# tsnorri/founder-sequences

Measured on AMD Instinct MI355X. Metric: alignment cells/s (m*n/T) through pBWT+DP, higher is better.
Workload: dtype u32

## Files before the change

### founder-sequences_amd/csrc/fseq_chainsort.hpp

```cpp
#pragma once

#include <type_traits>

#include "fseq_stream.hpp"
#include "fseq_types.hpp"

namespace fseq {

constexpr uint32_t CS_MAX_DIGIT_BITS = 9;
constexpr uint32_t CS_BINS = 1u << CS_MAX_DIGIT_BITS;
constexpr uint32_t CS_LEVELS = 16;

__host__ __device__ inline size_t chainsort_ws_words(uint32_t m)
{
	size_t const nblk = ((size_t) m + 63) / 64;
	return 8 * (size_t) m + CS_LEVELS * nblk + 64;
}

__device__ __forceinline__ uint64_t cs_match(uint32_t dg, bool in, uint32_t nbits)
{
	uint64_t mask = __ballot(in);
#pragma unroll
	for (uint32_t b = 0; b < CS_MAX_DIGIT_BITS; ++b)
		if (b < nbits)
		{
			uint64_t const bal = __ballot(in && ((dg >> b) & 1u));
			mask &= ((dg >> b) & 1u) ? bal : ~bal;
		}
	return mask;
}

__device__ __forceinline__ uint32_t cs_below(uint64_t mask)
{
	return (uint32_t) __builtin_amdgcn_mbcnt_hi((uint32_t) (mask >> 32), __builtin_amdgcn_mbcnt_lo((uint32_t) mask, 0u));
}

constexpr uint32_t P2_CLS_CAP = 11264;

constexpr uint32_t P2_RUN_CAP = 8832;
constexpr uint32_t P2_CLS_BITS = 14;
static_assert(P2_CLS_CAP <= (1u << P2_CLS_BITS), "a class of a reduced block fits a descriptor");

struct Pass2Lds {
	uint32_t scan[ST / WAVE + 1];
	uint32_t grp;
	union {
		struct {
			uint32_t hist[ST / WAVE][CS_BINS];
			uint32_t total[CS_BINS];
			uint16_t cls[P2_CLS_CAP];
		};
		struct {
			uint32_t off[P2_RUN_CAP + 1];
			uint32_t dsc[P2_RUN_CAP];
		};
	};
};

__host__ __device__ inline size_t pass2_lds_bytes() { return carve_bytes(1, sizeof(Pass2Lds)); }

__host__ __device__ inline size_t pass2_ws_r(uint32_t m) { return (((size_t) m + 1) / 2 + 3) & ~size_t(3); }
__host__ __device__ inline size_t pass2_ws_words(uint32_t m)
{
	size_t const nblk = ((size_t) m + 63) / 64;
	return pass2_ws_r(m) + 2 * (size_t) m + 2 * (size_t) m + 4 * (size_t) m + ((CS_LEVELS * nblk + 64 + 3) & ~size_t(3));
}
struct Pass2Ws {
	uint16_t *r;
	uint32_t *bufB, *bufA;
	uint4 *rec;
	uint32_t *tab;
};
__device__ __forceinline__ Pass2Ws pass2_ws(uint32_t *w, uint32_t m)
{
	Pass2Ws W;
	W.r = reinterpret_cast<uint16_t *>(w);
	W.bufB = w + pass2_ws_r(m);
	W.bufA = W.bufB + 2u * (size_t) m;
	W.rec = reinterpret_cast<uint4 *>(W.bufA + 2u * (size_t) m);
	W.tab = W.bufA + 6u * (size_t) m;
	return W;
}

__device__ __forceinline__ void pass2_digits(uint32_t D, uint32_t &npass, uint32_t &db)
{
	uint32_t bits = 1;
	while (bits < 32u && ((D - 1u) >> bits) != 0u) ++bits;
	npass = (bits + CS_MAX_DIGIT_BITS - 1u) / CS_MAX_DIGIT_BITS;
	db = (bits + npass - 1u) / npass;
}

template <typename PairT, uint32_t U = 4, typename Load0, typename KeyOf, typename Lds>
__device__ __forceinline__ void pass2_sort(uint32_t cnt, uint32_t npass, uint32_t db, Load0 load0, KeyOf key_of, PairT none, PairT *bufA, PairT *bufB, Lds &S)
{
	uint32_t const tid = threadIdx.x, lane = lane_id();
	uint32_t const wave = __builtin_amdgcn_readfirstlane(tid >> 6);
	constexpr uint32_t NW = ST / WAVE;
	uint32_t const nbins = 1u << db;
	uint32_t const per = ((cnt + NW - 1u) / NW + 63u) & ~63u;
	uint32_t const c_lo = min(cnt, wave * per), c_hi = min(cnt, c_lo + per);
	for (uint32_t p = 0; p < npass; ++p)
	{
		uint32_t const shift = p * db;
		bool const first = p == 0;
		PairT const *src = ((npass - p) & 1u) ? bufA : bufB;
		PairT *dst = ((npass - p) & 1u) ? bufB : bufA;
		auto load = [&](uint32_t i) -> PairT { return first ? load0(i) : src[i]; };
// ... 56 lines not shown
		}
#pragma unroll
		for (uint32_t u = 0; u < UB; ++u)
		{
			uint32_t const blk = b0 + u * NW, i = blk * 64u + lane;
			if (blk >= nblk) break;
			uint32_t const pre = wave_incl_max(v[u]);
			uint32_t const rev = (uint32_t) __builtin_amdgcn_ds_bpermute((int) ((63u - lane) << 2), (int) v[u]);
			uint32_t const sufr = wave_incl_max(rev);
			uint32_t const sufn = (uint32_t) __builtin_amdgcn_ds_bpermute((int) ((62u - min(lane, 62u)) << 2), (int) sufr);
			if (i < m) rec[i] = make_uint4(a[u], v[u], pre, lane == 63u ? 0u : sufn);
			if (lane == 63u) tab[blk] = pre;
		}
	}
	__syncthreads();
	for (uint32_t j = tid; j + 1u < nblk; j += ST) rec[j * 64u + 63u].w = tab[j + 1u];
	for (uint32_t k = 1; k < CS_LEVELS && (1u << k) <= nblk; ++k)
	{
		uint32_t const *lo = tab + (size_t) (k - 1u) * nblk;
		uint32_t *hi = tab + (size_t) k * nblk;
		for (uint32_t j = tid; j + (1u << k) <= nblk; j += ST) hi[j] = max(lo[j], lo[j + (1u << (k - 1u))]);
		__syncthreads();
	}
	__syncthreads();
}

__device__ __forceinline__ uint32_t pass2_range_max(uint32_t lo, uint32_t hi, uint4 const *rec, uint32_t const *tab, uint32_t nblk, uint32_t const *__restrict__ d0)
{
	uint32_t const bl = lo >> 6, bh = hi >> 6;
	uint4 const rc = rec[hi], q = rec[lo - 1u];
	uint32_t const pz = q.z, sv = q.w;
	uint32_t dv = max(sv, rc.z);
	if (bh > bl + 1u)
	{
		uint32_t const k = 31u - (uint32_t) __builtin_clz(bh - bl - 1u);
		uint32_t const *t = tab + (size_t) k * nblk;
		dv = max(dv, max(t[bl + 1u], t[bh - (1u << k)]));
	}
	if (bl == bh)
	{
		if ((lo & 63u) == 0u || rc.z > pz) dv = rc.z;
		else if ((hi & 63u) == 63u || sv > rc.w) dv = sv;
		else
		{
			dv = rc.y;
			for (uint32_t i = lo; i < hi; ++i) dv = max(dv, d0[i]);
		}
	}
	return dv;
}

__device__ __forceinline__ bool pass2_runs(
	uint32_t m, uint32_t const *__restrict__ kd, uint32_t D, Pass2Ws const &W, Pass2Lds &S, uint32_t run_cap, uint32_t *nrun,
	uint32_t const *__restrict__ a0, uint32_t const *__restrict__ d0, uint32_t *__restrict__ a1, uint32_t *__restrict__ d1)
{
	uint32_t const tid = threadIdx.x, lane = lane_id();
	uint32_t const wave = __builtin_amdgcn_readfirstlane(tid >> 6);
	constexpr uint32_t NW = ST / WAVE;
	uint16_t const *__restrict__ r = W.r;
	uint32_t pb = 1;
	while (pb < 32u && ((m - 1u) >> pb) != 0u) ++pb;
	uint32_t const pmask = (1u << pb) - 1u;
	uint32_t const nblk = (m + 63u) / 64u;
	uint32_t const per = ((m + NW - 1u) / NW + 63u) & ~63u;
	uint32_t const c_lo = min(m, wave * per), c_hi = min(m, c_lo + per);
	constexpr uint32_t U = 4;

	uint32_t npass, db;
	pass2_digits(D, npass, db);
	uint2 *const bufA = reinterpret_cast<uint2 *>(W.bufA), *const bufB = reinterpret_cast<uint2 *>(W.bufB);
	uint32_t *const pos_order = reinterpret_cast<uint32_t *>((npass & 1u) ? bufA : bufB);
	uint32_t R = 0, wbase = 0;
	for (uint32_t sweep = 0; sweep < 2u; ++sweep)
	{
		uint32_t prev = 0xFFFFFFFFu;
		if (c_lo > 0u && c_lo < c_hi) prev = (uint32_t) S.cls[r[c_lo - 1u]];
		uint32_t k0 = wbase;
		for (uint32_t i0 = c_lo; i0 < c_hi; i0 += 64u * U)
		{
			uint32_t rv[U];
#pragma unroll
			for (uint32_t u = 0; u < U; ++u) { uint32_t const i = i0 + u * 64u + lane; rv[u] = i < c_hi ? (uint32_t) r[i] : 0u; }
#pragma unroll
			for (uint32_t u = 0; u < U; ++u)
			{
				uint32_t const i = i0 + u * 64u + lane;
				if (i0 + u * 64u >= c_hi) break;
				bool const in = i < c_hi;
				uint32_t const cl = (uint32_t) S.cls[rv[u]];
				uint32_t const up = shfl_up_u32(cl, 1);
				bool const head = in && cl != (lane ? up : prev);
				uint64_t const heads = __ballot(head);
				if (sweep)
				{
					uint32_t const k = k0 + cs_below(heads);
					if (head)
					{
						pos_order[2u * k] = (cl << pb) | i;
						if (k) pos_order[2u * k - 1u] = i;
					}
				}
				k0 += (uint32_t) __popcll(heads);
				prev = readlane_u32(cl, 63);
			}
		}
		if (sweep) break;
		uint32_t const before = block_excl_add<ST>(lane == 0u ? k0 : 0u, S.scan, &R);
		wbase = __builtin_amdgcn_readfirstlane(before);
		*nrun = R;
		if (R > run_cap) return false;
	}
	if (tid == 0u) pos_order[2u * R - 1u] = m;
	__syncthreads();

	pass2_sort<uint2>(R, npass, db, [&](uint32_t i) -> uint2 { return reinterpret_cast<uint2 const *>(pos_order)[i]; },
	                  [&](uint2 x) -> uint32_t { return x.x >> pb; }, make_uint2(0u, 0u), bufA, bufB, S);
	{
		uint32_t const q = (R + ST - 1u) / ST, j0 = min(R, tid * q), j1 = min(R, j0 + q);
		uint32_t sum = 0;
		for (uint32_t j = j0; j < j1; ++j) { uint2 const x = bufB[j]; sum += x.y - (x.x & pmask); }
		uint32_t all;
		uint32_t at = block_excl_add<ST>(sum, S.scan, &all);
		for (uint32_t j = j0; j < j1; ++j) { uint2 const x = bufB[j]; S.off[j] = at; S.dsc[j] = x.x; at += x.y - (x.x & pmask); }
		if (tid == 0u) S.off[R] = m;
	}
	__syncthreads();

	uint32_t top = 1;
	while (top * 2u < R) top *= 2u;
	for (uint32_t p0 = tid; p0 < m; p0 += ST * U)
	{
		uint32_t jj[U], hh[U], av[U], dv[U];
#pragma unroll
		for (uint32_t u = 0; u < U; ++u)
		{
			uint32_t const p = min(p0 + u * ST, m - 1u);
			uint32_t j = 0;
			for (uint32_t step = top; step; step >>= 1) { uint32_t const t = j + step; if (t < R && S.off[t] <= p) j = t; }
			jj[u] = j;
			hh[u] = (S.dsc[j] & pmask) + (p - S.off[j]);
		}
#pragma unroll
		for (uint32_t u = 0; u < U; ++u) { av[u] = a0[hh[u]]; dv[u] = d0[hh[u]]; }
#pragma unroll
		for (uint32_t u = 0; u < U; ++u)
		{
			uint32_t const p = p0 + u * ST, j = jj[u];
			if (p >= m) break;
			if (S.off[j] == p)
			{
				uint32_t const me = S.dsc[j], pv = j ? S.dsc[j - 1u] : 0u;
				if (j == 0u || (pv >> pb) != (me >> pb)) dv[u] = kd[me >> pb];
				else dv[u] = pass2_range_max((pv & pmask) + (p - S.off[j - 1u]), hh[u], W.rec, W.tab, nblk, d0);
			}
			a1[p] = av[u];
			d1[p] = dv[u];
		}
	}
	__syncthreads();
	return true;
}

template <bool P4>
__device__ __forceinline__ void pass2_place(
	uint32_t m, uint32_t const *__restrict__ kd, std::conditional_t<P4, uint32_t, uint2> const *perm, uint4 const *rec, uint32_t const *tab,
	uint32_t const *__restrict__ d0, uint32_t *__restrict__ a1, uint32_t *__restrict__ d1)
{
	uint32_t const tid = threadIdx.x, lane = lane_id();
	using PairT = std::conditional_t<P4, uint32_t, uint2>;
	uint32_t pb = 1;
	while (pb < 32u && ((m - 1u) >> pb) != 0u) ++pb;
	uint32_t const pmask = pb < 32u ? (1u << pb) - 1u : 0xFFFFFFFFu;
	auto key_of = [&](PairT pr) -> uint32_t { if constexpr (P4) return pr >> pb; else return pr.x; };
	auto pos_of = [&](PairT pr) -> uint32_t { if constexpr (P4) return pr & pmask; else return pr.y; };
	uint32_t const nblk = (m + 63u) / 64u;
	{
		constexpr uint32_t U = 4;
		for (uint32_t p0 = tid; p0 < m; p0 += ST * U)
		{
			uint2 me[U], pv[U];
#pragma unroll
			for (uint32_t u = 0; u < U; ++u)
			{
				uint32_t const p = min(p0 + u * ST, m - 1u);
				PairT const pm_ = perm[p], pp_ = perm[p ? p - 1u : 0u];
				me[u] = make_uint2(key_of(pm_), pos_of(pm_));
				pv[u] = make_uint2(key_of(pp_), pos_of(pp_));
			}
			uint4 rc[U];
			uint32_t z0[U], w0[U], kdv[U], t0[U], t1[U];
#pragma unroll
			for (uint32_t u = 0; u < U; ++u)
			{
				uint32_t const p = p0 + u * ST;
				bool const first = p == 0u || pv[u].x != me[u].x;
				uint32_t const lo = pv[u].y + 1u, hi = me[u].y;
				uint32_t const bl = lo >> 6, bh = hi >> 6;
				rc[u] = rec[hi];
				z0[u] = 0u; w0[u] = 0u; kdv[u] = 0u; t0[u] = 0u; t1[u] = 0u;
				if (lane == 0u && !first) { uint4 const q = rec[pv[u].y]; z0[u] = q.z; w0[u] = q.w; }
				if (p < m && first) kdv[u] = kd[me[u].x];
				if (p < m && !first && bh > bl + 1u)
				{
					uint32_t const k = 31u - (uint32_t) __builtin_clz(bh - bl - 1u);
					uint32_t const *t = tab + (size_t) k * nblk;
					t0[u] = t[bl + 1u];
					t1[u] = t[bh - (1u << k)];
				}
			}
#pragma unroll
			for (uint32_t u = 0; u < U; ++u)
			{
// ... 14 lines not shown
						else if ((hi & 63u) == 63u || sv > rc[u].w) dv = sv;
						else
						{
							dv = rc[u].y;
							for (uint32_t i = lo; i < hi; i += 4u)
							{
								uint32_t const x0 = d0[i], x1 = i + 1u < hi ? d0[i + 1u] : 0u;
								uint32_t const x2 = i + 2u < hi ? d0[i + 2u] : 0u, x3 = i + 3u < hi ? d0[i + 3u] : 0u;
								dv = max(dv, max(max(x0, x1), max(x2, x3)));
							}
						}
					}
					a1[p] = rc[u].x;
					d1[p] = first ? kdv[u] : dv;
				}
			}
		}
	}
	__syncthreads();
}

template <bool P4>
__device__ __forceinline__ void pass2_step(
	uint32_t m, uint32_t const *__restrict__ kd, uint32_t D, Pass2Ws const &W, Pass2Lds &S,
	uint32_t const *__restrict__ d0, uint32_t *__restrict__ a1, uint32_t *__restrict__ d1)
{
	using PairT = std::conditional_t<P4, uint32_t, uint2>;
	uint32_t pb = 1;
	while (pb < 32u && ((m - 1u) >> pb) != 0u) ++pb;
	auto mk = [&](uint32_t key, uint32_t pos) -> PairT { if constexpr (P4) return (key << pb) | pos; else return make_uint2(key, pos); };
	auto key_of = [&](PairT pr) -> uint32_t { if constexpr (P4) return pr >> pb; else return pr.x; };
	uint16_t const *__restrict__ r = W.r;

	uint32_t npass, db;
	pass2_digits(D, npass, db);
	pass2_sort<PairT>(m, npass, db, [&](uint32_t i) -> PairT { return mk((uint32_t) S.cls[r[i]], i); }, key_of, mk(0u, 0u),
	                  reinterpret_cast<PairT *>(W.bufA), reinterpret_cast<PairT *>(W.bufB), S);
	pass2_place<P4>(m, kd, reinterpret_cast<PairT const *>(W.bufB), W.rec, W.tab, d0, a1, d1);
}

__global__ __launch_bounds__(ST) void k_chain_snap_grouped(
	uint32_t const *__restrict__ bstate_a, uint32_t const *__restrict__ bstate_d, uint32_t const *__restrict__ rank, uint32_t m,
	uint32_t const *__restrict__ task_blk, uint32_t const *__restrict__ cls, uint32_t const *__restrict__ headd, uint32_t const *__restrict__ ncls,
	uint32_t cap, uint2 const *__restrict__ grps, uint32_t ngrp, uint32_t *__restrict__ grp_next, uint32_t *__restrict__ snap_a,
	uint32_t *__restrict__ snap_d, uint32_t *ws, uint32_t run_cap, uint32_t *__restrict__ stats,
	uint16_t const *hand_keys, uint32_t const *hand_flag, uint32_t *hand_stats)
{
	extern __shared__ __attribute__((aligned(16))) char smem[];
	Pass2Lds &S = *reinterpret_cast<Pass2Lds *>(smem);
	uint32_t const tid = threadIdx.x;
	Pass2Ws const W0 = pass2_ws(ws + (size_t) blockIdx.x * pass2_ws_words(m), m);
	uint32_t pbits = 1;
	while (pbits < 32u && ((m - 1u) >> pbits) != 0u) ++pbits;
	for (;;)
	{
		if (tid == 0) S.grp = atomicAdd(grp_next, 1u);
		__syncthreads();
		uint32_t const g = S.grp;
		__syncthreads();
		if (g >= ngrp) break;
		uint2 const gr = grps[g];
		uint32_t const blk = task_blk[gr.x];
		size_t const sb = (size_t) blk * m;
		uint32_t const *a0 = bstate_a + sb, *d0 = bstate_d + sb;
		bool const handed = hand_keys != nullptr && hand_flag[blk] != 0u;
		Pass2Ws W = W0;
		if (handed) W.r = const_cast<uint16_t *>(hand_keys) + sb;
		if (hand_stats && tid == 0) atomicAdd(hand_stats + (handed ? 0 : 1), 1u);
		bool have_r = false;
		for (uint32_t task = gr.x; task < gr.x + gr.y; ++task)
		{
			uint32_t const D = ncls[task];
			if (D == 0xFFFFFFFFu) continue;
			size_t const ob = (size_t) task * m;
			if (D == 0u)
			{
				for (uint32_t i = tid; i < m; i += ST) { snap_a[ob + i] = a0[i]; snap_d[ob + i] = d0[i]; }
				if (tid == 0) atomicAdd(stats + 2, 1u);
				continue;
			}
			if (!have_r)
			{
				constexpr uint32_t U = 4;
				if (!handed)
					for (uint32_t i0 = tid; i0 < m; i0 += ST * U)
					{
						uint32_t rv[U];
#pragma unroll
						for (uint32_t u = 0; u < U; ++u) { uint32_t const i = i0 + u * ST; rv[u] = i < m ? rank[sb + a0[i]] : 0u; }
#pragma unroll
						for (uint32_t u = 0; u < U; ++u) { uint32_t const i = i0 + u * ST; if (i < m) W.r[i] = (uint16_t) rv[u]; }
					}
				pass2_records(m, a0, d0, W.rec, W.tab);
				have_r = true;
			}
			for (uint32_t j = tid; j < cap; j += ST) S.cls[j] = (uint16_t) cls[(size_t) task * cap + j];
			__syncthreads();
			uint32_t kb = 1;
			while (kb < 32u && ((D - 1u) >> kb) != 0u) ++kb;
			bool const p4 = kb + pbits <= 32u;
			uint32_t const *kd = headd + (size_t) task * cap;
			uint32_t nrun = 0;
			bool const by_runs = run_cap != 0u && P2_CLS_BITS + pbits <= 32u && pass2_runs(m, kd, D, W, S, run_cap, &nrun, a0, d0, snap_a + ob, snap_d + ob);
			if (!by_runs)
			{
				if (p4) pass2_step<true>(m, kd, D, W, S, d0, snap_a + ob, snap_d + ob);
				else pass2_step<false>(m, kd, D, W, S, d0, snap_a + ob, snap_d + ob);
			}
			if (tid == 0)
			{
				atomicAdd(stats + (by_runs ? 0 : 1), 1u);
				if (nrun)
				{
					atomicMax(stats + 3, nrun);
					atomicAdd(stats + 4 + min(P2_HIST - 1u, nrun > 1u ? 32u - (uint32_t) __builtin_clz(nrun - 1u) : 0u), 1u);
				}
			}
		}
	}
}

constexpr uint32_t CM_PART = 1024;
constexpr uint32_t CM_WG = 256;


struct CmWg { uint32_t x, chain; bool ok; };
__device__ __forceinline__ CmWg cm_wg(ChainMultiArgs const &A)
{
	CmWg w;
	uint32_t const nx = gridDim.x, L = blockIdx.y * nx + blockIdx.x;
	uint32_t const xcd = L & 7u, slot = L >> 3;
	w.chain = (slot / nx) * 8u + xcd;
	w.x = slot % nx;
	w.ok = w.chain < A.nchains;
	return w;
}

__host__ __device__ inline uint32_t chainmulti_parts(uint32_t m) { return (m + CM_PART - 1u) / CM_PART; }
__host__ __device__ inline uint32_t chainmulti_passes(uint32_t m)
{
	uint32_t bits = 1;
	while (bits < 32u && ((m - 1u) >> bits) != 0u) ++bits;
	return (bits + CS_MAX_DIGIT_BITS - 1u) / CS_MAX_DIGIT_BITS;
}

struct ChainMultiGeom {
	uint32_t b, npass, db, nbins;
	uint32_t pb;
	bool p4;
	bool active;
	uint32_t *w;
	uint32_t const *a0, *d0;
	uint32_t *a1, *d1;
	uint2 *pairA, *pairB;
	uint32_t *pm, *sm, *tab;
	uint32_t *hist;
};

__device__ __forceinline__ ChainMultiGeom chainmulti_geom(ChainMultiArgs const &A, uint32_t chain)
{
	ChainMultiGeom g;
	uint32_t const grp = chain + A.grp0;
	uint32_t const b0 = grp * A.G, b1 = min(A.nb_total, b0 + A.G);
	g.b = b0 + A.step;
	g.active = g.b < b1 && (A.out_rank != nullptr || g.b + 1u < b1 || g.b + 1u == A.nb_total);
	uint32_t const nk = g.active ? A.nkeys[g.b] : 1u;
	uint32_t bits = 1;
	while (bits < 32u && ((nk - 1u) >> bits) != 0u) ++bits;
	g.npass = (bits + CS_MAX_DIGIT_BITS - 1u) / CS_MAX_DIGIT_BITS;
	g.db = (bits + g.npass - 1u) / g.npass;
	g.nbins = 1u << g.db;
// ... 241 lines not shown
			dv = g.d0[hi];
			for (uint32_t i = lo; i < hi; ++i) dv = max(dv, g.d0[i]);
		}
		else
		{
			dv = max(g.sm[lo], g.pm[hi]);
			if (bh > bl + 1u)
			{
				uint32_t const k = 31u - (uint32_t) __builtin_clz(bh - bl - 1u);
				uint32_t const *t = g.tab + (size_t) k * nblk;
				dv = max(dv, max(t[bl + 1u], t[bh - (1u << k)]));
			}
		}
	}
	g.a1[p] = row; g.d1[p] = dv;
	uint32_t const grp = wg.chain + A.grp0;
	uint32_t const b1 = min(A.nb_total, grp * A.G + A.G);
	if (A.out_state_a && (g.b + 1u < b1 || g.b + 1u == A.nb_total))
	{
		A.out_state_a[(size_t) (g.b + 1u) * m + p] = row; A.out_state_d[(size_t) (g.b + 1u) * m + p] = dv;
	}
}

__global__ __launch_bounds__(ST) void k_cm_emit(ChainMultiArgs const A, uint32_t steps_done)
{
	extern __shared__ __attribute__((aligned(16))) char smem[];
	Carver cv{smem};
	StreamLds &L = *cv.take<StreamLds>(1);
	uint32_t const chain = blockIdx.x, grp = chain + A.grp0, m = A.m;
	uint32_t const b0 = grp * A.G;
	if (b0 >= A.nb_total) return;
	uint32_t const b1 = min(A.nb_total, b0 + A.G);
	uint32_t const cur = (b1 - b0) & 1u;
	(void) steps_done;
	uint32_t const *w = A.ws + (size_t) chain * chainsort_ws_words(m);
	uint32_t const *a = w + (size_t) cur * 2u * m, *d = a + m;
	uint32_t const kstart = (uint32_t) ((uint64_t) b0 * A.cols_per_block);
	stream_emit_ranks(m, a, d, kstart, A.out_rank + (size_t) grp * m, A.out_keyd + (size_t) grp * m, A.out_nkeys + grp, L.red);
}

constexpr uint32_t CW_RUN_CAP = 16384;
constexpr uint32_t CW_RBLK = CW_RUN_CAP / 64;
constexpr uint32_t CW_RLEVELS = 9;
static_assert(CW_RUN_CAP % 64u == 0u && CW_RBLK <= (1u << (CW_RLEVELS - 1u)), "the table over the blocks of runs");

struct ChainWgLds {
	uint32_t scan[ST / WAVE + 1];
	union {
		struct {
			uint32_t hist[ST / WAVE][CS_BINS];
			uint32_t total[CS_BINS];
		};
		struct {
			uint32_t off[CW_RUN_CAP + 1];
			uint32_t dlt[CW_RUN_CAP];
		};
	};
};
static_assert(sizeof(ChainWgLds) + 16u <= 160u * 1024u, "a workgroup a CU");

__host__ __device__ inline size_t chainwg_lds_bytes() { return carve_bytes(1, sizeof(ChainWgLds)); }

__host__ __device__ inline size_t chainwg_ws_rows(uint32_t m) { return ((size_t) m + 3) & ~size_t(3); }
__host__ __device__ inline size_t chainwg_ws_tab(uint32_t m) { return (CS_LEVELS * (((size_t) m + 63) / 64) + 64 + 3) & ~size_t(3); }
__host__ __device__ inline size_t chainwg_ws_words(uint32_t m)
{
	return 13 * chainwg_ws_rows(m) + chainwg_ws_tab(m) + 5 * (size_t) (CW_RUN_CAP + 64) + (size_t) CW_RLEVELS * CW_RBLK;
}
struct ChainWgWs {
	uint4 *rec;
	uint32_t *bufB, *bufA, *state, *keys, *tab;
	uint32_t *rstart, *rmax, *rpre, *rsuf, *rhead, *rtab;
};
__device__ __forceinline__ ChainWgWs chainwg_ws(uint32_t *w, uint32_t m)
{
	size_t const M = chainwg_ws_rows(m);
	ChainWgWs W;
	W.rec = reinterpret_cast<uint4 *>(w);
	W.bufB = w + 4 * M; W.bufA = w + 6 * M;
	W.state = w + 8 * M;
	W.keys = w + 12 * M;
	W.tab = w + 13 * M;
	W.rstart = W.tab + chainwg_ws_tab(m);
	W.rmax = W.rstart + (CW_RUN_CAP + 64); W.rpre = W.rmax + (CW_RUN_CAP + 64); W.rsuf = W.rpre + (CW_RUN_CAP + 64);
	W.rhead = W.rsuf + (CW_RUN_CAP + 64);
	W.rtab = W.rhead + (CW_RUN_CAP + 64);
	return W;
}

__device__ __forceinline__ uint32_t chainwg_rmax(uint32_t const *rmax, uint32_t k)
{
	return __hip_atomic_load(rmax + k, __ATOMIC_RELAXED, __HIP_MEMORY_SCOPE_AGENT);
}

__device__ __forceinline__ uint32_t chainwg_run_max(uint32_t lo, uint32_t hi, uint32_t R, ChainWgWs const &W)
{
	uint32_t const bl = lo >> 6, bh = hi >> 6;
	if (bl == bh)
	{
		if ((lo & 63u) == 0u) return W.rpre[hi];
		if ((hi & 63u) == 63u || hi + 1u == R) return W.rsuf[lo];
		uint32_t v = 0;
		for (uint32_t k = lo; k <= hi; ++k) v = max(v, chainwg_rmax(W.rmax, k));
		return v;
	}
	uint32_t v = max(W.rsuf[lo], W.rpre[hi]);
	if (bh > bl + 1u)
	{
		uint32_t const k = 31u - (uint32_t) __builtin_clz(bh - bl - 1u);
		uint32_t const *t = W.rtab + (size_t) k * CW_RBLK;
		v = max(v, max(t[bl + 1u], t[bh - (1u << k)]));
	}
	return v;
}


constexpr uint32_t CW_U = 8;

__device__ __forceinline__ uint32_t chainwg_keys(uint32_t m, uint32_t const *__restrict__ rk, uint32_t const *a0, ChainWgWs const &W, ChainWgLds &S, uint16_t *hk,
                                                 uint32_t *R)
{
	uint32_t const tid = threadIdx.x, lane = lane_id();
	uint32_t const wave = __builtin_amdgcn_readfirstlane(tid >> 6);
	constexpr uint32_t NW = ST / WAVE;
	uint32_t const per = ((m + NW - 1u) / NW + 63u) & ~63u;
	uint32_t const c_lo = min(m, wave * per), c_hi = min(m, c_lo + per);
	uint32_t prev = 0xFFFFFFFFu;
	if (c_lo > 0u && c_lo < c_hi) prev = rk[a0[c_lo - 1u]];
	uint32_t k0 = 0;
	for (uint32_t i0 = c_lo; i0 < c_hi; i0 += 64u * CW_U)
	{
		uint32_t av[CW_U], kv[CW_U];
#pragma unroll
		for (uint32_t u = 0; u < CW_U; ++u) { uint32_t const i = i0 + u * 64u + lane; av[u] = i < c_hi ? a0[i] : 0u; }
#pragma unroll
		for (uint32_t u = 0; u < CW_U; ++u) { uint32_t const i = i0 + u * 64u + lane; kv[u] = i < c_hi ? rk[av[u]] : 0u; }
#pragma unroll
		for (uint32_t u = 0; u < CW_U; ++u)
		{
			uint32_t const i = i0 + u * 64u + lane;
			if (i0 + u * 64u >= c_hi) break;
			bool const in = i < c_hi;
			if (in) W.keys[i] = kv[u];
			if (hk && in) hk[i] = (uint16_t) kv[u];
			uint32_t const up = shfl_up_u32(kv[u], 1);
			k0 += (uint32_t) __popcll(__ballot(in && kv[u] != (lane ? up : prev)));
			prev = readlane_u32(kv[u], 63);
		}
	}
	uint32_t const before = block_excl_add<ST>(lane == 0u ? k0 : 0u, S.scan, R);
	__syncthreads();
	return __builtin_amdgcn_readfirstlane(before);
}

__device__ __forceinline__ void chainwg_runs(
	uint32_t m, uint32_t const *__restrict__ kd, uint32_t nk, ChainWgWs const &W, ChainWgLds &S, uint32_t R, uint32_t wbase,
	uint32_t const *a0, uint32_t const *d0, uint32_t *a1, uint32_t *d1)
{
	uint32_t const tid = threadIdx.x, lane = lane_id();
	uint32_t const wave = __builtin_amdgcn_readfirstlane(tid >> 6);
	constexpr uint32_t NW = ST / WAVE;
	uint32_t const *keys = W.keys;
	uint32_t pb = 1;
	while (pb < 32u && ((m - 1u) >> pb) != 0u) ++pb;
	uint32_t const pmask = (1u << pb) - 1u;
	uint32_t const per = ((m + NW - 1u) / NW + 63u) & ~63u;
	uint32_t const c_lo = min(m, wave * per), c_hi = min(m, c_lo + per);
	uint32_t npass, db;
	pass2_digits(nk, npass, db);
	uint2 *const bufA = reinterpret_cast<uint2 *>(W.bufA), *const bufB = reinterpret_cast<uint2 *>(W.bufB);
	uint2 *const pos_order = (npass & 1u) ? bufA : bufB;

	for (uint32_t k = tid; k < R; k += ST) W.rmax[k] = 0u;
	__syncthreads();
	{
		uint32_t prev = 0xFFFFFFFFu;
		if (c_lo > 0u && c_lo < c_hi) prev = keys[c_lo - 1u];
		uint32_t k0 = wbase;
		for (uint32_t i0 = c_lo; i0 < c_hi; i0 += 64u * CW_U)
		{
			uint32_t kv[CW_U], dv[CW_U];
#pragma unroll
			for (uint32_t u = 0; u < CW_U; ++u)
			{
				uint32_t const i = i0 + u * 64u + lane;
				kv[u] = i < c_hi ? keys[i] : 0u;
				dv[u] = i < c_hi ? d0[i] : 0u;
			}
#pragma unroll
			for (uint32_t u = 0; u < CW_U; ++u)
			{
				uint32_t const i = i0 + u * 64u + lane;
				if (i0 + u * 64u >= c_hi) break;
				bool const in = i < c_hi;
				uint32_t const up = shfl_up_u32(kv[u], 1);
				bool const head = in && kv[u] != (lane ? up : prev);
				uint64_t const heads = __ballot(head);
				uint32_t const k = k0 + cs_below(heads) + (head ? 1u : 0u) - 1u;
				if (head) { pos_order[k] = make_uint2((kv[u] << pb) | i, k); W.rstart[k] = i; }
				uint64_t const upto = heads & (lane == 63u ? ~0ull : ((2ull << lane) - 1ull));
				uint32_t const s0 = upto ? 63u - (uint32_t) __builtin_clzll(upto) : 0u;
				uint32_t v = dv[u];
#pragma unroll
				for (uint32_t o = 1; o < 64u; o <<= 1)
				{
					uint32_t const t = shfl_up_u32(v, (int) o);
					if (lane >= s0 + o) v = max(v, t);
				}
				uint64_t const ins = __ballot(in);
				bool const last = in && (lane == 63u || !((ins >> (lane + 1u)) & 1ull) || ((heads >> (lane + 1u)) & 1ull));
				if (last) atomicMax(&W.rmax[k], v);
				k0 += (uint32_t) __popcll(heads);
				prev = readlane_u32(kv[u], 63);
			}
		}
	}
	if (tid == 0u) W.rstart[R] = m;
	__syncthreads();

	uint32_t const nrb = (R + 63u) / 64u;
	for (uint32_t blk = wave; blk < nrb; blk += NW)
	{
		uint32_t const k = blk * 64u + lane;
		uint32_t const v = k < R ? chainwg_rmax(W.rmax, k) : 0u;
		uint32_t const pre = wave_incl_max(v);
		uint32_t const rev = (uint32_t) __builtin_amdgcn_ds_bpermute((int) ((63u - lane) << 2), (int) v);
		uint32_t const sufr = wave_incl_max(rev);
		uint32_t const suf = (uint32_t) __builtin_amdgcn_ds_bpermute((int) ((63u - lane) << 2), (int) sufr);
		if (k < R) { W.rpre[k] = pre; W.rsuf[k] = suf; }
		if (lane == 63u) W.rtab[blk] = pre;
	}
	__syncthreads();
	for (uint32_t k = 1; k < CW_RLEVELS && (1u << k) <= nrb; ++k)
	{
		uint32_t const *lo = W.rtab + (size_t) (k - 1u) * CW_RBLK;
		uint32_t *hi = W.rtab + (size_t) k * CW_RBLK;
		for (uint32_t j = tid; j + (1u << k) <= nrb; j += ST) hi[j] = max(lo[j], lo[j + (1u << (k - 1u))]);
		__syncthreads();
	}

	pass2_sort<uint2>(R, npass, db, [&](uint32_t i) -> uint2 { return pos_order[i]; }, [&](uint2 x) -> uint32_t { return x.x >> pb; },
	                  make_uint2(0u, 0u), bufA, bufB, S);
	{
		constexpr uint32_t Q = CW_RUN_CAP / ST;
		static_assert(Q * ST == CW_RUN_CAP, "a thread's runs");
		uint32_t const q = (R + ST - 1u) / ST, j0 = min(R, tid * q), j1 = min(R, j0 + q);
		uint32_t st[Q], len[Q];
#pragma unroll
		for (uint32_t t = 0; t < Q; ++t)
		{
			uint2 const x = j0 + t < j1 ? bufB[j0 + t] : make_uint2(0u, 0u);
			st[t] = x.x & pmask; len[t] = x.y;
		}
#pragma unroll
		for (uint32_t t = 0; t < Q; ++t) len[t] = j0 + t < j1 ? W.rstart[len[t] + 1u] - st[t] : 0u;
		uint32_t sum = 0;
#pragma unroll
		for (uint32_t t = 0; t < Q; ++t) sum += len[t];
		uint32_t all;
		uint32_t at = block_excl_add<ST>(sum, S.scan, &all);
#pragma unroll
		for (uint32_t t = 0; t < Q; ++t)
			if (j0 + t < j1) { S.off[j0 + t] = at; S.dlt[j0 + t] = st[t] - at; at += len[t]; }
		if (tid == 0u) S.off[R] = m;
	}

	{
		constexpr uint32_t UH = 4;
		for (uint32_t j0 = tid; j0 < R; j0 += ST * UH)
		{
			uint2 me[UH], pv[UH];
			uint32_t hv[UH];
#pragma unroll
			for (uint32_t u = 0; u < UH; ++u)
			{
				uint32_t const j = min(j0 + u * ST, R - 1u);
				me[u] = bufB[j]; pv[u] = bufB[j ? j - 1u : 0u];
			}
#pragma unroll
			for (uint32_t u = 0; u < UH; ++u)
			{
				uint32_t const j = j0 + u * ST;
				hv[u] = 0u;
				if (j >= R) continue;
				if (j == 0u || (pv[u].x >> pb) != (me[u].x >> pb)) hv[u] = kd[me[u].x >> pb];
				else
				{
					hv[u] = d0[me[u].x & pmask];
					uint32_t const k_lo = pv[u].y + 1u, k_me = me[u].y;
					if (k_lo < k_me) hv[u] = max(hv[u], chainwg_run_max(k_lo, k_me - 1u, R, W));
				}
			}
#pragma unroll
			for (uint32_t u = 0; u < UH; ++u) { uint32_t const j = j0 + u * ST; if (j < R) W.rhead[j] = hv[u]; }
		}
	}
	__syncthreads();

	uint32_t top = 1;
	while (top * 2u < R) top *= 2u;
	for (uint32_t p0 = tid; p0 < m; p0 += ST * CW_U)
	{
		uint32_t jh[CW_U], hh[CW_U], av[CW_U], dv[CW_U];
#pragma unroll
		for (uint32_t u = 0; u < CW_U; ++u)
		{
			uint32_t const p = min(p0 + u * ST, m - 1u);
			uint32_t j = 0;
			for (uint32_t step = top; step; step >>= 1) { uint32_t const t = j + step; if (t < R && S.off[t] <= p) j = t; }
			hh[u] = p + S.dlt[j];
			jh[u] = S.off[j] == p ? j : 0xFFFFFFFFu;
		}
#pragma unroll
		for (uint32_t u = 0; u < CW_U; ++u) { av[u] = a0[hh[u]]; dv[u] = jh[u] != 0xFFFFFFFFu ? W.rhead[jh[u]] : d0[hh[u]]; }
#pragma unroll
		for (uint32_t u = 0; u < CW_U; ++u)
		{
			uint32_t const p = p0 + u * ST;
			if (p < m) { a1[p] = av[u]; d1[p] = dv[u]; }
		}
	}
	__syncthreads();
}

template <bool P4>
__device__ __forceinline__ void chainwg_sort(
	uint32_t m, uint32_t const *__restrict__ rk, uint32_t const *__restrict__ kd, uint32_t nk, ChainWgWs const &W, ChainWgLds &S, bool ident, uint32_t kstart,
	uint32_t const *a0, uint32_t const *d0, uint32_t *a1, uint32_t *d1)
{
	using PairT = std::conditional_t<P4, uint32_t, uint2>;
	uint32_t pb = 1;
	while (pb < 32u && ((m - 1u) >> pb) != 0u) ++pb;
	uint32_t const pmask = pb < 32u ? (1u << pb) - 1u : 0xFFFFFFFFu;
	auto mk = [&](uint32_t key, uint32_t pos) -> PairT { if constexpr (P4) return (key << pb) | pos; else return make_uint2(key, pos); };
	auto key_of = [&](PairT pr) -> uint32_t { if constexpr (P4) return pr >> pb; else return pr.x; };
	auto pos_of = [&](PairT pr) -> uint32_t { if constexpr (P4) return pr & pmask; else return pr.y; };
	uint32_t npass, db;
	pass2_digits(nk, npass, db);
	PairT *const bufA = reinterpret_cast<PairT *>(W.bufA), *const bufB = reinterpret_cast<PairT *>(W.bufB);
	if (ident)
	{
		pass2_sort<PairT, CW_U>(m, npass, db, [&](uint32_t i) -> PairT { return mk(rk[i], i); }, key_of, mk(0u, 0u), bufA, bufB, S);
		for (uint32_t p0 = threadIdx.x; p0 < m; p0 += ST * CW_U)
		{
			PairT me[CW_U], pv[CW_U];
			uint32_t dv[CW_U];
#pragma unroll
			for (uint32_t u = 0; u < CW_U; ++u) { uint32_t const p = min(p0 + u * ST, m - 1u); me[u] = bufB[p]; pv[u] = bufB[p ? p - 1u : 0u]; }
#pragma unroll
			for (uint32_t u = 0; u < CW_U; ++u)
			{
				uint32_t const p = p0 + u * ST;
				dv[u] = (p < m && (p == 0u || key_of(pv[u]) != key_of(me[u]))) ? kd[key_of(me[u])] : kstart;
			}
#pragma unroll
			for (uint32_t u = 0; u < CW_U; ++u) { uint32_t const p = p0 + u * ST; if (p < m) { a1[p] = pos_of(me[u]); d1[p] = dv[u]; } }
		}
		__syncthreads();
		return;
	}
	uint32_t const *keys = W.keys;
	pass2_records(m, a0, d0, W.rec, W.tab);
	pass2_sort<PairT, CW_U>(m, npass, db, [&](uint32_t i) -> PairT { return mk(keys[i], i); }, key_of, mk(0u, 0u), bufA, bufB, S);
	pass2_place<P4>(m, kd, bufB, W.rec, W.tab, d0, a1, d1);
}

__global__ __launch_bounds__(ST) void k_chain_wg(ChainMultiArgs const A, uint32_t *ws, uint32_t run_cap, uint32_t *stats)
{
	extern __shared__ __attribute__((aligned(16))) char smem[];
	ChainWgLds &S = *reinterpret_cast<ChainWgLds *>(smem);
	uint32_t const tid = threadIdx.x, m = A.m;
	ChainWgWs const W = chainwg_ws(ws + (size_t) blockIdx.x * chainwg_ws_words(m), m);
	uint32_t pbits = 1;
	while (pbits < 32u && ((m - 1u) >> pbits) != 0u) ++pbits;
	for (uint32_t chain = blockIdx.x; chain < A.nchains; chain += gridDim.x)
	{
		uint32_t const grp = chain + A.grp0;
		uint32_t const b0 = grp * A.G;
		if (b0 >= A.nb_total) continue;
		uint32_t const b1 = min(A.nb_total, b0 + A.G);
		uint32_t const kstart = (uint32_t) ((uint64_t) b0 * A.cols_per_block);
		bool ident = A.start_a == nullptr;
		uint32_t const *a0 = ident ? nullptr : A.start_a + (size_t) grp * m, *d0 = ident ? nullptr : A.start_d + (size_t) grp * m;
		if (A.out_state_a)
			for (uint32_t i = tid; i < m; i += ST)
			{
				A.out_state_a[(size_t) b0 * m + i] = ident ? i : a0[i];
				A.out_state_d[(size_t) b0 * m + i] = ident ? kstart : d0[i];
			}
		uint32_t pp = 0;
		for (uint32_t b = b0; b < b1; ++b)
		{
			bool const keep = b + 1u < b1 || b + 1u == A.nb_total;
			if (!A.out_rank && !keep) break;
			uint32_t *a1, *d1;
			if (A.out_state_a && keep) { a1 = A.out_state_a + (size_t) (b + 1u) * m; d1 = A.out_state_d + (size_t) (b + 1u) * m; }
			else { a1 = W.state + (size_t) pp * 2u * chainwg_ws_rows(m); d1 = a1 + chainwg_ws_rows(m); pp ^= 1u; }
			uint32_t const *rk = A.rank + (size_t) b * m, *kd = A.keyd + (size_t) b * m;
			uint32_t const nk = A.nkeys[b];
			uint32_t kb = 1;
			while (kb < 32u && ((nk - 1u) >> kb) != 0u) ++kb;
			bool const p4 = kb + pbits <= 32u;
			uint32_t nrun = 0;
			bool by_runs = false;
			uint16_t *const hk = A.hand_keys && A.out_state_a && !A.out_rank && !ident && nk <= 65536u ? A.hand_keys + (size_t) b * m : nullptr;
			if (!ident)
			{
				uint32_t R = 0;
				uint32_t const wbase = chainwg_keys(m, rk, a0, W, S, hk, &R);
				bool const may = run_cap != 0u && p4;
				nrun = may ? R : 0u;
				by_runs = may && R <= run_cap;
				if (by_runs) chainwg_runs(m, kd, nk, W, S, R, wbase, a0, d0, a1, d1);
			}
			if (!by_runs)
			{
				if (p4) chainwg_sort<true>(m, rk, kd, nk, W, S, ident, kstart, a0, d0, a1, d1);
				else chainwg_sort<false>(m, rk, kd, nk, W, S, ident, kstart, a0, d0, a1, d1);
			}
			if (hk && tid == 0u) A.hand_flag[b] = 1u;
			if (stats && tid == 0)
			{
				atomicAdd(stats + (ident ? 2 : by_runs ? 0 : 1), 1u);
				if (nrun)
				{
					atomicMax(stats + 3, nrun);
					atomicAdd(stats + 4 + min(P2_HIST - 1u, nrun > 1u ? 32u - (uint32_t) __builtin_clz(nrun - 1u) : 0u), 1u);
				}
			}
			ident = false;
			a0 = a1; d0 = d1;
		}
		if (A.out_rank)
		{
			stream_emit_ranks(m, a0, d0, kstart, A.out_rank + (size_t) grp * m, A.out_keyd + (size_t) grp * m, A.out_nkeys + grp, S.scan);
			__syncthreads();
		}
	}
}

}
```

Baseline: 2327 billion.

## Replace run binary search with LDS select bitmap and vectorize run-head sweep

Replaces the per-row binary search over run offsets with a bitmap of run starts plus per-64-row prefix counts in LDS, so each row finds its run with a popcount and mbcnt. In pass2_runs it also computes run-head d values once per run in a separate pass, and it reads the 16-bit class keys eight at a time with uint4 loads when aligned. Optional timestamp instrumentation is added behind a macro. The cost is extra LDS, an atomicOr per run and another barrier and sweep.

```diff
diff --git a/founder-sequences_amd/csrc/fseq_chainsort.hpp b/founder-sequences_amd/csrc/fseq_chainsort.hpp
--- a/founder-sequences_amd/csrc/fseq_chainsort.hpp
+++ b/founder-sequences_amd/csrc/fseq_chainsort.hpp
@@ -35,11 +35,69 @@
 	return (uint32_t) __builtin_amdgcn_mbcnt_hi((uint32_t) (mask >> 32), __builtin_amdgcn_mbcnt_lo((uint32_t) mask, 0u));
 }
 
+#ifdef FSEQ_RUN_STAMPS
+struct RunStamps {
+	unsigned long long last, acc[8];
+	uint32_t steps;
+	__device__ __forceinline__ void clear() { for (int i = 0; i < 8; ++i) acc[i] = 0; steps = 0; }
+	__device__ __forceinline__ void start() { last = __builtin_amdgcn_s_memrealtime(); }
+	__device__ __forceinline__ void mark(int part) { unsigned long long const t = __builtin_amdgcn_s_memrealtime(); acc[part] += t - last; last = t; }
+};
+#define FSEQ_RS_PARAM , RunStamps &rs
+#define FSEQ_RS_ARG , rs
+#define FSEQ_RS_MARK(part) rs.mark(part)
+#else
+#define FSEQ_RS_PARAM
+#define FSEQ_RS_ARG
+#define FSEQ_RS_MARK(part)
+#endif
+
 constexpr uint32_t P2_CLS_CAP = 11264;
 
 constexpr uint32_t P2_RUN_CAP = 8832;
 constexpr uint32_t P2_CLS_BITS = 14;
 static_assert(P2_CLS_CAP <= (1u << P2_CLS_BITS), "a class of a reduced block fits a descriptor");
+
+constexpr uint32_t CW_U = 8;
+
+constexpr uint32_t SEL_ROWS = 1u << 18;
+struct RunSelect {
+	uint32_t bits[SEL_ROWS / 32];
+	uint16_t pre[SEL_ROWS / 64];
+};
+
+__device__ __forceinline__ void sel_clear(RunSelect &B, uint32_t m)
+{
+	for (uint32_t w = threadIdx.x; w < 2u * ((m + 63u) / 64u); w += ST) B.bits[w] = 0u;
+}
+__device__ __forceinline__ void sel_set(RunSelect &B, uint32_t p) { atomicOr(&B.bits[p >> 5], 1u << (p & 31u)); }
+__device__ __forceinline__ void sel_scan(RunSelect &B, uint32_t m, uint32_t *scan)
+{
+	__syncthreads();
+	constexpr uint32_t Q = SEL_ROWS / 64u / ST;
+	uint32_t const nw = (m + 63u) / 64u, w0 = threadIdx.x * Q;
+	uint32_t c[Q], sum = 0;
+#pragma unroll
+	for (uint32_t t = 0; t < Q; ++t)
+	{
+		c[t] = w0 + t < nw ? (uint32_t) __popc(B.bits[2u * (w0 + t)]) + (uint32_t) __popc(B.bits[2u * (w0 + t) + 1u]) : 0u;
+		sum += c[t];
+	}
+	uint32_t all;
+	uint32_t at = block_excl_add<ST>(sum, scan, &all);
+#pragma unroll
+	for (uint32_t t = 0; t < Q; ++t)
+		if (w0 + t < nw) { B.pre[w0 + t] = (uint16_t) at; at += c[t]; }
+}
+__device__ __forceinline__ uint32_t sel_run(RunSelect const &B, uint32_t p, uint32_t m, bool *head)
+{
+	uint32_t const w = __builtin_amdgcn_readfirstlane(min(p, m - 1u) >> 6);
+	uint32_t const lo = __builtin_amdgcn_readfirstlane(B.bits[2u * w]), hi = __builtin_amdgcn_readfirstlane(B.bits[2u * w + 1u]);
+	uint32_t const lane = lane_id();
+	bool const h = (((lane < 32u ? lo : hi) >> (lane & 31u)) & 1u) != 0u;
+	*head = h;
+	return (uint32_t) B.pre[w] + (uint32_t) __builtin_amdgcn_mbcnt_hi(hi, __builtin_amdgcn_mbcnt_lo(lo, 0u)) + (h ? 1u : 0u) - 1u;
+}
 
 struct Pass2Lds {
 	uint32_t scan[ST / WAVE + 1];
@@ -51,8 +109,8 @@
 			uint16_t cls[P2_CLS_CAP];
 		};
 		struct {
-			uint32_t off[P2_RUN_CAP + 1];
-			uint32_t dsc[P2_RUN_CAP];
+			uint32_t dlt[P2_RUN_CAP];
+			RunSelect sel;
 		};
 	};
 };
@@ -215,7 +273,7 @@
 
 __device__ __forceinline__ bool pass2_runs(
 	uint32_t m, uint32_t const *__restrict__ kd, uint32_t D, Pass2Ws const &W, Pass2Lds &S, uint32_t run_cap, uint32_t *nrun,
-	uint32_t const *__restrict__ a0, uint32_t const *__restrict__ d0, uint32_t *__restrict__ a1, uint32_t *__restrict__ d1)
+	uint32_t const *__restrict__ a0, uint32_t const *__restrict__ d0, uint32_t *__restrict__ a1, uint32_t *__restrict__ d1 FSEQ_RS_PARAM)
 {
 	uint32_t const tid = threadIdx.x, lane = lane_id();
 	uint32_t const wave = __builtin_amdgcn_readfirstlane(tid >> 6);
@@ -229,6 +287,8 @@
 	uint32_t const c_lo = min(m, wave * per), c_hi = min(m, c_lo + per);
 	constexpr uint32_t U = 4;
 
+	bool const vec = (reinterpret_cast<uintptr_t>(r) & 15u) == 0u;
+	constexpr uint32_t PC = 8, UV = 4;
 	uint32_t npass, db;
 	pass2_digits(D, npass, db);
 	uint2 *const bufA = reinterpret_cast<uint2 *>(W.bufA), *const bufB = reinterpret_cast<uint2 *>(W.bufB);
@@ -239,7 +299,59 @@
 		uint32_t prev = 0xFFFFFFFFu;
 		if (c_lo > 0u && c_lo < c_hi) prev = (uint32_t) S.cls[r[c_lo - 1u]];
 		uint32_t k0 = wbase;
-		for (uint32_t i0 = c_lo; i0 < c_hi; i0 += 64u * U)
+		for (uint32_t i0 = c_lo; vec && i0 < c_hi; i0 += 64u * PC * UV)
+		{
+			uint4 rv[UV];
+#pragma unroll
+			for (uint32_t u = 0; u < UV; ++u)
+			{
+				uint32_t const ib = i0 + (u * 64u + lane) * PC;
+				rv[u] = make_uint4(0u, 0u, 0u, 0u);
+				if (ib + PC <= c_hi) rv[u] = *reinterpret_cast<uint4 const *>(r + ib);
+				else if (ib < c_hi)
+				{
+					uint32_t x[PC / 2u] = {0u, 0u, 0u, 0u};
+#pragma unroll
+					for (uint32_t e = 0; e < PC; ++e)
+						if (ib + e < c_hi) x[e >> 1] |= (uint32_t) r[ib + e] << (16u * (e & 1u));
+					rv[u] = make_uint4(x[0], x[1], x[2], x[3]);
+				}
+			}
+#pragma unroll
+			for (uint32_t u = 0; u < UV; ++u)
+			{
+				if (i0 + u * 64u * PC >= c_hi) break;
+				uint32_t const ib = i0 + (u * 64u + lane) * PC;
+				uint32_t const x[PC / 2u] = {rv[u].x, rv[u].y, rv[u].z, rv[u].w};
+				uint32_t cl[PC];
+#pragma unroll
+				for (uint32_t e = 0; e < PC; ++e) cl[e] = (uint32_t) S.cls[(x[e >> 1] >> (16u * (e & 1u))) & 0xFFFFu];
+				uint32_t const up = shfl_up_u32(cl[PC - 1u], 1);
+				uint32_t front = lane ? up : prev, hm = 0;
+#pragma unroll
+				for (uint32_t e = 0; e < PC; ++e)
+				{
+					if (ib + e < c_hi && cl[e] != front) hm |= 1u << e;
+					front = cl[e];
+				}
+				uint32_t const cnt = (uint32_t) __popc(hm), inc = wave_incl_add(cnt);
+				if (sweep)
+				{
+					uint32_t k = k0 + inc - cnt;
+#pragma unroll
+					for (uint32_t e = 0; e < PC; ++e)
+						if ((hm >> e) & 1u)
+						{
+							pos_order[2u * k] = (cl[e] << pb) | (ib + e);
+							if (k) pos_order[2u * k - 1u] = ib + e;
+							++k;
+						}
+				}
+				k0 += readlane_u32(inc, 63);
+				prev = readlane_u32(cl[PC - 1u], 63);
+			}
+		}
+		for (uint32_t i0 = c_lo; !vec && i0 < c_hi; i0 += 64u * U)
 		{
 			uint32_t rv[U];
 #pragma unroll
@@ -272,55 +384,87 @@
 		wbase = __builtin_amdgcn_readfirstlane(before);
 		*nrun = R;
 		if (R > run_cap) return false;
+		FSEQ_RS_MARK(1);
 	}
 	if (tid == 0u) pos_order[2u * R - 1u] = m;
 	__syncthreads();
+	FSEQ_RS_MARK(2);
 
 	pass2_sort<uint2>(R, npass, db, [&](uint32_t i) -> uint2 { return reinterpret_cast<uint2 const *>(pos_order)[i]; },
 	                  [&](uint2 x) -> uint32_t { return x.x >> pb; }, make_uint2(0u, 0u), bufA, bufB, S);
+	FSEQ_RS_MARK(3);
 	{
 		uint32_t const q = (R + ST - 1u) / ST, j0 = min(R, tid * q), j1 = min(R, j0 + q);
 		uint32_t sum = 0;
 		for (uint32_t j = j0; j < j1; ++j) { uint2 const x = bufB[j]; sum += x.y - (x.x & pmask); }
+		sel_clear(S.sel, m);
 		uint32_t all;
 		uint32_t at = block_excl_add<ST>(sum, S.scan, &all);
-		for (uint32_t j = j0; j < j1; ++j) { uint2 const x = bufB[j]; S.off[j] = at; S.dsc[j] = x.x; at += x.y - (x.x & pmask); }
-		if (tid == 0u) S.off[R] = m;
-	}
+		for (uint32_t j = j0; j < j1; ++j)
+		{
+			uint2 const x = bufB[j];
+			S.dlt[j] = (x.x & pmask) - at; sel_set(S.sel, at);
+			at += x.y - (x.x & pmask);
+		}
+		sel_scan(S.sel, m, S.scan);
+	}
+#ifdef FSEQ_RUN_STAMPS
 	__syncthreads();
-
-	uint32_t top = 1;
-	while (top * 2u < R) top *= 2u;
-	for (uint32_t p0 = tid; p0 < m; p0 += ST * U)
-	{
-		uint32_t jj[U], hh[U], av[U], dv[U];
-#pragma unroll
-		for (uint32_t u = 0; u < U; ++u)
-		{
-			uint32_t const p = min(p0 + u * ST, m - 1u);
-			uint32_t j = 0;
-			for (uint32_t step = top; step; step >>= 1) { uint32_t const t = j + step; if (t < R && S.off[t] <= p) j = t; }
-			jj[u] = j;
-			hh[u] = (S.dsc[j] & pmask) + (p - S.off[j]);
-		}
-#pragma unroll
-		for (uint32_t u = 0; u < U; ++u) { av[u] = a0[hh[u]]; dv[u] = d0[hh[u]]; }
-#pragma unroll
-		for (uint32_t u = 0; u < U; ++u)
-		{
-			uint32_t const p = p0 + u * ST, j = jj[u];
-			if (p >= m) break;
-			if (S.off[j] == p)
-			{
-				uint32_t const me = S.dsc[j], pv = j ? S.dsc[j - 1u] : 0u;
-				if (j == 0u || (pv >> pb) != (me >> pb)) dv[u] = kd[me >> pb];
-				else dv[u] = pass2_range_max((pv & pmask) + (p - S.off[j - 1u]), hh[u], W.rec, W.tab, nblk, d0);
-			}
-			a1[p] = av[u];
-			d1[p] = dv[u];
+#endif
+	FSEQ_RS_MARK(4);
+
+	uint32_t *const rhead = reinterpret_cast<uint32_t *>(bufA);
+	{
+		constexpr uint32_t UH = 4;
+		for (uint32_t j0 = tid; j0 < R; j0 += ST * UH)
+		{
+			uint2 me[UH], pv[UH];
+			uint32_t hv[UH];
+#pragma unroll
+			for (uint32_t u = 0; u < UH; ++u)
+			{
+				uint32_t const j = min(j0 + u * ST, R - 1u);
+				me[u] = bufB[j]; pv[u] = bufB[j ? j - 1u : 0u];
+			}
+#pragma unroll
+			for (uint32_t u = 0; u < UH; ++u)
+			{
+				uint32_t const j = j0 + u * ST;
+				hv[u] = 0u;
+				if (j >= R) continue;
+				if (j == 0u || (pv[u].x >> pb) != (me[u].x >> pb)) hv[u] = kd[me[u].x >> pb];
+				else hv[u] = pass2_range_max(pv[u].y, me[u].x & pmask, W.rec, W.tab, nblk, d0);
+			}
+#pragma unroll
+			for (uint32_t u = 0; u < UH; ++u) { uint32_t const j = j0 + u * ST; if (j < R) rhead[j] = hv[u]; }
 		}
 	}
 	__syncthreads();
+	FSEQ_RS_MARK(7);
+
+	for (uint32_t p0 = tid; p0 < m; p0 += ST * CW_U)
+	{
+		uint32_t jh[CW_U], hh[CW_U], av[CW_U], dv[CW_U];
+#pragma unroll
+		for (uint32_t u = 0; u < CW_U; ++u)
+		{
+			uint32_t const p = p0 + u * ST;
+			bool head;
+			uint32_t const j = sel_run(S.sel, p, m, &head);
+			hh[u] = p < m ? p + S.dlt[j] : 0u;
+			jh[u] = head && p < m ? j : 0xFFFFFFFFu;
+		}
+#pragma unroll
+		for (uint32_t u = 0; u < CW_U; ++u) { av[u] = a0[hh[u]]; dv[u] = jh[u] != 0xFFFFFFFFu ? rhead[jh[u]] : d0[hh[u]]; }
+#pragma unroll
+		for (uint32_t u = 0; u < CW_U; ++u)
+		{
+			uint32_t const p = p0 + u * ST;
+			if (p < m) { a1[p] = av[u]; d1[p] = dv[u]; }
+		}
+	}
+	__syncthreads();
+	FSEQ_RS_MARK(5);
 	return true;
 }
 
@@ -441,6 +585,10 @@
 	Pass2Ws const W0 = pass2_ws(ws + (size_t) blockIdx.x * pass2_ws_words(m), m);
 	uint32_t pbits = 1;
 	while (pbits < 32u && ((m - 1u) >> pbits) != 0u) ++pbits;
+#ifdef FSEQ_RUN_STAMPS
+	RunStamps rs;
+	uint32_t rs_groups = 0;
+#endif
 	for (;;)
 	{
 		if (tid == 0) S.grp = atomicAdd(grp_next, 1u);
@@ -457,6 +605,11 @@
 		if (handed) W.r = const_cast<uint16_t *>(hand_keys) + sb;
 		if (hand_stats && tid == 0) atomicAdd(hand_stats + (handed ? 0 : 1), 1u);
 		bool have_r = false;
+#ifdef FSEQ_RUN_STAMPS
+		rs.clear();
+		uint32_t rs_sorted = 0;
+		unsigned long long rs_runs = 0;
+#endif
 		for (uint32_t task = gr.x; task < gr.x + gr.y; ++task)
 		{
 			uint32_t const D = ncls[task];
@@ -480,17 +633,31 @@
 #pragma unroll
 						for (uint32_t u = 0; u < U; ++u) { uint32_t const i = i0 + u * ST; if (i < m) W.r[i] = (uint16_t) rv[u]; }
 					}
+#ifdef FSEQ_RUN_STAMPS
+				__syncthreads();
+				rs.start();
+#endif
 				pass2_records(m, a0, d0, W.rec, W.tab);
+				FSEQ_RS_MARK(6);
 				have_r = true;
 			}
+#ifdef FSEQ_RUN_STAMPS
+			RunStamps const rs_before = rs;
+			rs.start();
+#endif
 			for (uint32_t j = tid; j < cap; j += ST) S.cls[j] = (uint16_t) cls[(size_t) task * cap + j];
 			__syncthreads();
+			FSEQ_RS_MARK(0);
 			uint32_t kb = 1;
 			while (kb < 32u && ((D - 1u) >> kb) != 0u) ++kb;
 			bool const p4 = kb + pbits <= 32u;
 			uint32_t const *kd = headd + (size_t) task * cap;
 			uint32_t nrun = 0;
-			bool const by_runs = run_cap != 0u && P2_CLS_BITS + pbits <= 32u && pass2_runs(m, kd, D, W, S, run_cap, &nrun, a0, d0, snap_a + ob, snap_d + ob);
+			bool const by_runs = run_cap != 0u && P2_CLS_BITS + pbits <= 32u && pass2_runs(m, kd, D, W, S, run_cap, &nrun, a0, d0, snap_a + ob, snap_d + ob FSEQ_RS_ARG);
+#ifdef FSEQ_RUN_STAMPS
+			if (by_runs) { ++rs.steps; rs_runs += nrun; }
+			else { rs = rs_before; ++rs_sorted; }
+#endif
 			if (!by_runs)
 			{
 				if (p4) pass2_step<true>(m, kd, D, W, S, d0, snap_a + ob, snap_d + ob);
@@ -506,6 +673,13 @@
 				}
 			}
 		}
+#ifdef FSEQ_RUN_STAMPS
+		if (tid == 0 && (blockIdx.x & 63u) == 0u && rs.steps != 0u && rs_groups++ < 3u)
+			printf("p2 run stamps workgroup %u block %u (%u rows, %s keys, %u tasks by runs of %llu runs on average, %u sorted): records %llu, per task by runs: class table %llu, "
+			       "sweep 0 %llu, sweep 1 %llu, descriptor sort %llu, prefix sums %llu, heads %llu, output sweep %llu (x 10 ns)\n",
+			       blockIdx.x, blk, m, handed ? "handed-over" : "gathered", rs.steps, rs_runs / rs.steps, rs_sorted, rs.acc[6], rs.acc[0] / rs.steps, rs.acc[1] / rs.steps,
+			       rs.acc[2] / rs.steps, rs.acc[3] / rs.steps, rs.acc[4] / rs.steps, rs.acc[7] / rs.steps, rs.acc[5] / rs.steps);
+#endif
 	}
 }
 
@@ -853,7 +1027,10 @@
 			uint32_t total[CS_BINS];
 		};
 		struct {
-			uint32_t off[CW_RUN_CAP + 1];
+			union {
+				RunSelect sel;
+				uint32_t off[CW_RUN_CAP + 1];
+			};
 			uint32_t dlt[CW_RUN_CAP];
 		};
 	};
@@ -916,7 +1093,6 @@
 }
 
 
-constexpr uint32_t CW_U = 8;
 
 __device__ __forceinline__ uint32_t chainwg_keys(uint32_t m, uint32_t const *__restrict__ rk, uint32_t const *a0, ChainWgWs const &W, ChainWgLds &S, uint16_t *hk,
                                                  uint32_t *R)
@@ -956,7 +1132,7 @@
 
 __device__ __forceinline__ void chainwg_runs(
 	uint32_t m, uint32_t const *__restrict__ kd, uint32_t nk, ChainWgWs const &W, ChainWgLds &S, uint32_t R, uint32_t wbase,
-	uint32_t const *a0, uint32_t const *d0, uint32_t *a1, uint32_t *d1)
+	uint32_t const *a0, uint32_t const *d0, uint32_t *a1, uint32_t *d1 FSEQ_RS_PARAM)
 {
 	uint32_t const tid = threadIdx.x, lane = lane_id();
 	uint32_t const wave = __builtin_amdgcn_readfirstlane(tid >> 6);
@@ -971,6 +1147,7 @@
 	pass2_digits(nk, npass, db);
 	uint2 *const bufA = reinterpret_cast<uint2 *>(W.bufA), *const bufB = reinterpret_cast<uint2 *>(W.bufB);
 	uint2 *const pos_order = (npass & 1u) ? bufA : bufB;
+	bool const by_select = m <= SEL_ROWS;
 
 	for (uint32_t k = tid; k < R; k += ST) W.rmax[k] = 0u;
 	__syncthreads();
@@ -1018,6 +1195,7 @@
 	}
 	if (tid == 0u) W.rstart[R] = m;
 	__syncthreads();
+	FSEQ_RS_MARK(1);
 
 	uint32_t const nrb = (R + 63u) / 64u;
 	for (uint32_t blk = wave; blk < nrb; blk += NW)
@@ -1039,9 +1217,11 @@
 		for (uint32_t j = tid; j + (1u << k) <= nrb; j += ST) hi[j] = max(lo[j], lo[j + (1u << (k - 1u))]);
 		__syncthreads();
 	}
+	FSEQ_RS_MARK(2);
 
 	pass2_sort<uint2>(R, npass, db, [&](uint32_t i) -> uint2 { return pos_order[i]; }, [&](uint2 x) -> uint32_t { return x.x >> pb; },
 	                  make_uint2(0u, 0u), bufA, bufB, S);
+	FSEQ_RS_MARK(3);
 	{
 		constexpr uint32_t Q = CW_RUN_CAP / ST;
 		static_assert(Q * ST == CW_RUN_CAP, "a thread's runs");
@@ -1058,13 +1238,23 @@
 		uint32_t sum = 0;
 #pragma unroll
 		for (uint32_t t = 0; t < Q; ++t) sum += len[t];
+		if (by_select) sel_clear(S.sel, m);
 		uint32_t all;
 		uint32_t at = block_excl_add<ST>(sum, S.scan, &all);
 #pragma unroll
 		for (uint32_t t = 0; t < Q; ++t)
-			if (j0 + t < j1) { S.off[j0 + t] = at; S.dlt[j0 + t] = st[t] - at; at += len[t]; }
-		if (tid == 0u) S.off[R] = m;
-	}
+			if (j0 + t < j1)
+			{
+				if (by_select) sel_set(S.sel, at); else S.off[j0 + t] = at;
+				S.dlt[j0 + t] = st[t] - at; at += len[t];
+			}
+		if (by_select) sel_scan(S.sel, m, S.scan);
+		else if (tid == 0u) S.off[R] = m;
+	}
+#ifdef FSEQ_RUN_STAMPS
+	__syncthreads();
+#endif
+	FSEQ_RS_MARK(4);
 
 	{
 		constexpr uint32_t UH = 4;
@@ -1097,20 +1287,36 @@
 		}
 	}
 	__syncthreads();
+	FSEQ_RS_MARK(5);
 
 	uint32_t top = 1;
 	while (top * 2u < R) top *= 2u;
 	for (uint32_t p0 = tid; p0 < m; p0 += ST * CW_U)
 	{
 		uint32_t jh[CW_U], hh[CW_U], av[CW_U], dv[CW_U];
-#pragma unroll
-		for (uint32_t u = 0; u < CW_U; ++u)
-		{
-			uint32_t const p = min(p0 + u * ST, m - 1u);
-			uint32_t j = 0;
-			for (uint32_t step = top; step; step >>= 1) { uint32_t const t = j + step; if (t < R && S.off[t] <= p) j = t; }
-			hh[u] = p + S.dlt[j];
-			jh[u] = S.off[j] == p ? j : 0xFFFFFFFFu;
+		if (by_select)
+		{
+#pragma unroll
+			for (uint32_t u = 0; u < CW_U; ++u)
+			{
+				uint32_t const p = p0 + u * ST;
+				bool head;
+				uint32_t const j = sel_run(S.sel, p, m, &head);
+				hh[u] = p < m ? p + S.dlt[j] : 0u;
+				jh[u] = head && p < m ? j : 0xFFFFFFFFu;
+			}
+		}
+		else
+		{
+#pragma unroll
+			for (uint32_t u = 0; u < CW_U; ++u)
+			{
+				uint32_t const p = min(p0 + u * ST, m - 1u);
+				uint32_t j = 0;
+				for (uint32_t step = top; step; step >>= 1) { uint32_t const t = j + step; if (t < R && S.off[t] <= p) j = t; }
+				hh[u] = p + S.dlt[j];
+				jh[u] = S.off[j] == p ? j : 0xFFFFFFFFu;
+			}
 		}
 #pragma unroll
 		for (uint32_t u = 0; u < CW_U; ++u) { av[u] = a0[hh[u]]; dv[u] = jh[u] != 0xFFFFFFFFu ? W.rhead[jh[u]] : d0[hh[u]]; }
@@ -1122,6 +1328,7 @@
 		}
 	}
 	__syncthreads();
+	FSEQ_RS_MARK(6);
 }
 
 template <bool P4>
@@ -1174,6 +1381,9 @@
 	ChainWgWs const W = chainwg_ws(ws + (size_t) blockIdx.x * chainwg_ws_words(m), m);
 	uint32_t pbits = 1;
 	while (pbits < 32u && ((m - 1u) >> pbits) != 0u) ++pbits;
+#ifdef FSEQ_RUN_STAMPS
+	RunStamps rs;
+#endif
 	for (uint32_t chain = blockIdx.x; chain < A.nchains; chain += gridDim.x)
 	{
 		uint32_t const grp = chain + A.grp0;
@@ -1181,6 +1391,10 @@
 		if (b0 >= A.nb_total) continue;
 		uint32_t const b1 = min(A.nb_total, b0 + A.G);
 		uint32_t const kstart = (uint32_t) ((uint64_t) b0 * A.cols_per_block);
+#ifdef FSEQ_RUN_STAMPS
+		rs.clear();
+		unsigned long long rs_runs = 0;
+#endif
 		bool ident = A.start_a == nullptr;
 		uint32_t const *a0 = ident ? nullptr : A.start_a + (size_t) grp * m, *d0 = ident ? nullptr : A.start_d + (size_t) grp * m;
 		if (A.out_state_a)
@@ -1208,11 +1422,20 @@
 			if (!ident)
 			{
 				uint32_t R = 0;
+#ifdef FSEQ_RUN_STAMPS
+				RunStamps const rs_before = rs;
+				rs.start();
+#endif
 				uint32_t const wbase = chainwg_keys(m, rk, a0, W, S, hk, &R);
+				FSEQ_RS_MARK(0);
 				bool const may = run_cap != 0u && p4;
 				nrun = may ? R : 0u;
 				by_runs = may && R <= run_cap;
-				if (by_runs) chainwg_runs(m, kd, nk, W, S, R, wbase, a0, d0, a1, d1);
+				if (by_runs) chainwg_runs(m, kd, nk, W, S, R, wbase, a0, d0, a1, d1 FSEQ_RS_ARG);
+#ifdef FSEQ_RUN_STAMPS
+				if (by_runs) { ++rs.steps; rs_runs += R; }
+				else rs = rs_before;
+#endif
 			}
 			if (!by_runs)
 			{
@@ -1232,6 +1455,13 @@
 			ident = false;
 			a0 = a1; d0 = d1;
 		}
+#ifdef FSEQ_RUN_STAMPS
+		if (tid == 0 && (blockIdx.x & 63u) == 0u && chain == blockIdx.x && rs.steps != 0u)
+			printf("cw run stamps workgroup %u chain %u (%u rows, %s, %u steps by runs of %llu runs on average), per step by runs: keys and run count %llu, "
+			       "a descriptors and maxima %llu, b table %llu, c descriptor sort %llu, prefix sums %llu, d heads %llu, e new order %llu (x 10 ns)\n",
+			       blockIdx.x, chain, m, A.out_rank ? "composition" : "expansion", rs.steps, rs_runs / rs.steps, rs.acc[0] / rs.steps, rs.acc[1] / rs.steps,
+			       rs.acc[2] / rs.steps, rs.acc[3] / rs.steps, rs.acc[4] / rs.steps, rs.acc[5] / rs.steps, rs.acc[6] / rs.steps);
+#endif
 		if (A.out_rank)
 		{
 			stream_emit_ranks(m, a0, d0, kstart, A.out_rank + (size_t) grp * m, A.out_keyd + (size_t) grp * m, A.out_nkeys + grp, S.scan);
```

New measurement: 2477 billion, median of 6. 1.06x the previous value.
